# theAdamColton/spiht

Hardware: AMD Instinct MI355X
Metric: Mpixels/sec encode+decode at fixed bpp; bitstream-exact vs Rust ref (higher is better)
Workload: dtype f64 DWT / int32 bit-plane coding; 1 GPU; cfg2 image (1920x1080 RGB, bior2.2 reflect level 7, q=50, 0.5 bpp) x 256 per GPU (cfg4 shard), encode+decode, HBM-resident; images_per_gpu=256, distinct_images_per_gpu=256, seeds=1000 + global image index, streams=1, images_per_launch=256, decoder_waves=8, max_bits=1036800

## Files before the change

include/spiht_hip.h:

```cpp
#ifndef SPIHT_HIP_H
#define SPIHT_HIP_H

#include <stdint.h>

#ifdef __cplusplus
extern "C" {
#endif

enum {
    SPIHT_OK = 0,
    SPIHT_ERR_LL = 1,
    SPIHT_ERR_EMPTY = 2,
    SPIHT_ERR_SHAPE = 3,
    SPIHT_ERR_CAPACITY = 4,
    SPIHT_ERR_HIP = 5,
    SPIHT_ERR_ARG = 6,
    SPIHT_ERR_MAGNITUDE = 7,
    SPIHT_ERR_INTERNAL = 8,
    SPIHT_ERR_TOO_LARGE = 9,
    SPIHT_ERR_NOMEM = 10
};

enum { SPIHT_MODE_REFLECT = 0, SPIHT_MODE_SYMMETRIC = 1, SPIHT_MODE_PERIODIC = 2, SPIHT_MODE_ZERO = 3,
       SPIHT_MODE_CONSTANT = 4,
// ... 389 lines not shown
int spiht_convert_batch_flt(spiht_ctx *ctx, int kind, const double *d_in, int64_t B, int64_t c, int64_t rec_h, int64_t rec_w,
                            int64_t H, int64_t W, void *d_out, const int64_t *out_strides);
int spiht_decode_image_batch_flt(spiht_ctx *ctx, int kind, const uint8_t *d_data, uint64_t slot_stride, const uint64_t *d_nbytes,
                                 const uint8_t *d_max_n, int64_t B, int64_t c, int64_t H, int64_t W, int wavelet, int mode,
                                 int level, double q_scale, const double *channel_mults, void *d_img_out,
                                 const int64_t *out_strides, int32_t *d_rec);
int spiht_decode_image_host_flt(spiht_ctx *ctx, int kind, const uint8_t *data, uint64_t nbytes, uint8_t n, int64_t c, int64_t H,
                                int64_t W, int wavelet, int mode, int level, double q_scale, const double *channel_mults,
                                void *img_out, const int64_t *strides);
int spiht_dequant_idwt_flags_batch_flt(spiht_ctx *ctx, int kind, const int32_t *d_rec, const uint32_t *d_flags, int64_t B,
                                       int64_t c, int64_t H, int64_t W, int wavelet, int mode, int level, double q_scale,
                                       const double *channel_mults, void *d_img_out, const int64_t *out_strides);
int spiht_dequant_idwt_reduced_batch_flt(spiht_ctx *ctx, int kind, const int32_t *d_rec, int64_t B, int64_t c, int64_t H,
                                         int64_t W, int wavelet, int mode, int level, double q_scale,
                                         const double *channel_mults, void *d_img_out, const int64_t *out_strides, int reduce);
int spiht_decode_image_reduced_batch_flt(spiht_ctx *ctx, int kind, const uint8_t *d_data, uint64_t slot_stride,
                                         const uint64_t *d_nbytes, const uint8_t *d_max_n, int64_t B, int64_t c, int64_t H,
                                         int64_t W, int wavelet, int mode, int level, double q_scale,
                                         const double *channel_mults, void *d_img_out, const int64_t *out_strides,
                                         int32_t *d_rec, int reduce);
int spiht_decode_image_reduced_host_flt(spiht_ctx *ctx, int kind, const uint8_t *data, uint64_t nbytes, uint8_t n, int64_t c,
                                        int64_t H, int64_t W, int wavelet, int mode, int level, double q_scale,
                                        const double *channel_mults, void *img_out, const int64_t *strides, int reduce);
int spiht_tile_paste_f32s(spiht_ctx *ctx, const float *d_tiles, int64_t c, int64_t rh, int64_t rw, int64_t H, int64_t W,
                          int64_t th, int64_t tw, int64_t i0, int64_t i1, int64_t j0, int64_t j1, int64_t y0, int64_t x0,
                          int64_t wh, int64_t ww, float *d_out, const int64_t *out_strides);
int spiht_tile_mosaic_f32(spiht_ctx *ctx, const float *d_tiles, int64_t c, int64_t rh, int64_t rw, int64_t oy, int64_t ox,
                          int64_t H, int64_t W, int64_t th, int64_t tw, int64_t i0, int64_t i1, int64_t j0, int64_t j1,
                          int64_t y0, int64_t x0, int64_t wh, int64_t ww, float *d_out, const int64_t *out_strides);
int spiht_tile_blend_flt(spiht_ctx *ctx, int kind, const double *d_tiles, int64_t c, int64_t rh, int64_t rw, int64_t H, int64_t W,
                         int64_t th, int64_t tw, int64_t m, int64_t i0, int64_t i1, int64_t j0, int64_t j1, int64_t y0,
                         int64_t x0, int64_t wh, int64_t ww, void *d_out, const int64_t *out_strides);

#ifdef __cplusplus
}
#endif
#endif
```

spiht_amd/_lib.py:

```python
import ctypes as C
import os
import threading

_HERE = os.path.dirname(os.path.abspath(__file__))
LIB_PATH = os.environ.get("SPIHT_HIP_LIB") or os.path.join(_HERE, "libspiht_hip.so")

OK, ERR_LL, ERR_EMPTY, ERR_SHAPE, ERR_CAPACITY, ERR_HIP, ERR_ARG, ERR_MAGNITUDE, ERR_INTERNAL, ERR_TOO_LARGE, \
    ERR_NOMEM = range(11)

MODES = {"reflect": 0, "symmetric": 1, "periodic": 2, "zero": 3, "constant": 4}


class SpihtHipError(RuntimeError):
    """A HIP runtime failure or an internal guard of libspiht_hip."""


class PanicException(BaseException):
    """Counterpart of pyo3_runtime.PanicException, which the reference raises when the Rust core panics
    (assert!(ll_h > 1), encoder_decoder.rs:160-161; out-of-bounds index; unwrap on an empty array).
    Like PyO3's, it derives from BaseException."""


_lib = None
_lib_lock = threading.Lock()
# ... 12 lines not shown
    "spiht_dev_upload", "spiht_dev_download", "spiht_dev_memset", "spiht_dev_copy",
    "spiht_idwt_coarse_batch_f64", "spiht_idwt_level1_batch_f64", "spiht_idwt_level1_flags_batch_f64", "spiht_idwt_approx_shape",
    "spiht_encode_image_host_f64", "spiht_encode_image_host_f32", "spiht_decode_image_host_f64",
    "spiht_dequant_idwt_host_f64",
    "spiht_comm_unique_id", "spiht_comm_create", "spiht_comm_destroy", "spiht_comm_info", "spiht_gather_streams", "spiht_gather_row_offsets",
    "spiht_comm_barrier", "spiht_comm_allreduce_max_f64", "spiht_rccl_library", "spiht_ctx_lock", "spiht_ctx_unlock",
    "spiht_pipeline_create", "spiht_pipeline_create_on", "spiht_pipeline_destroy", "spiht_pipeline_info", "spiht_pipeline_set_color3", "spiht_pipeline_submit",
    "spiht_pipeline_submit_gather", "spiht_pipeline_flush", "spiht_pipeline_synchronize", "spiht_pipeline_contexts",
    "spiht_geometry_mode", "spiht_wavelet_taps", "spiht_ctx_set_option", "spiht_ctx_get_option", "spiht_ctx_wide_stats", "spiht_l1_flags_words", "spiht_decode_lists_flags_batch_i32", "spiht_dequant_idwt_flags_batch_f64",
    "spiht_encode_image_batch_u8", "spiht_decode_image_batch_u8", "spiht_encode_image_host_u8", "spiht_decode_image_host_u8",
    "spiht_dwt_pyramid_batch_u8", "spiht_dequant_idwt_flags_batch_u8", "spiht_idwt_level1_flags_batch_u8", "spiht_pipeline_submit_u8",
    "spiht_check_view_u8", "spiht_decode_with_metadata_batch_i32",
    "spiht_encode_image_batch_u16", "spiht_decode_image_batch_u16", "spiht_encode_image_host_u16", "spiht_decode_image_host_u16",
    "spiht_dwt_pyramid_batch_u16", "spiht_dequant_idwt_flags_batch_u16", "spiht_idwt_level1_flags_batch_u16", "spiht_pipeline_submit_u16",
    "spiht_check_view_u16",
    "spiht_reduced_shape",
    "spiht_dequant_idwt_reduced_batch_f64", "spiht_dequant_idwt_reduced_batch_u8", "spiht_dequant_idwt_reduced_batch_u16",
    "spiht_decode_image_reduced_batch_f64", "spiht_decode_image_reduced_batch_u8", "spiht_decode_image_reduced_batch_u16",
    "spiht_decode_image_reduced_host_f64", "spiht_decode_image_reduced_host_u8", "spiht_decode_image_reduced_host_u16",
    "spiht_sqerr_i32", "spiht_sse_f64", "spiht_sse_u8", "spiht_sse_u16",
    "spiht_tile_grid", "spiht_tile_cut_u8", "spiht_tile_cut_u16", "spiht_tile_cut_f32", "spiht_tile_cut_f64",
    "spiht_tile_paste_u8", "spiht_tile_paste_u16", "spiht_tile_paste_f32", "spiht_tile_paste_f64",
    "spiht_tile_pack", "spiht_tile_unpack",
    "spiht_tile_reduced_grid", "spiht_tile_mosaic_u8", "spiht_tile_mosaic_u16", "spiht_tile_mosaic_f64",
    "spiht_tile_prefix_slots", "spiht_sse_tiles_f64", "spiht_sse_tiles_u8", "spiht_sse_tiles_u16", "spiht_tile_allocate",
    "spiht_layer_pack", "spiht_layer_unpack",
    "spiht_sse_tiles_w_f64", "spiht_sse_tiles_w_u8", "spiht_sse_tiles_w_u16",
    "spiht_tile_allocate_target",
    "spiht_tile_cut_overlap_u8", "spiht_tile_cut_overlap_u16", "spiht_tile_cut_overlap_f32", "spiht_tile_cut_overlap_f64",
    "spiht_tile_blend_u8", "spiht_tile_blend_u16", "spiht_tile_blend_f64",
    "spiht_check_view_flt", "spiht_convert_batch_flt", "spiht_decode_image_batch_flt", "spiht_decode_image_host_flt",
    "spiht_dequant_idwt_flags_batch_flt", "spiht_dequant_idwt_reduced_batch_flt", "spiht_decode_image_reduced_batch_flt",
    "spiht_decode_image_reduced_host_flt", "spiht_tile_blend_flt", "spiht_tile_paste_f32s", "spiht_tile_mosaic_f32",
]


def lib():
    global _lib
    with _lib_lock:
        if _lib is not None:
            return _lib
        if not os.path.exists(LIB_PATH):
            raise ImportError(
                "libspiht_hip.so is missing (%s): build it with `python -c 'import __graft_entry__ as g; g.build()'` "
                "or `make -C spiht_amd/csrc`; spiht_amd has no CPU fallback" % LIB_PATH)
        try:
            L = C.CDLL(LIB_PATH)
        except OSError as e:
            raise ImportError("cannot load %s: %s" % (LIB_PATH, e))
        i64, u64, u8, i32 = C.c_int64, C.c_uint64, C.c_uint8, C.c_int
        vp = C.c_void_p
        L.spiht_strerror.restype = C.c_char_p
        L.spiht_strerror.argtypes = [i32]
        L.spiht_last_hip_error.restype = C.c_char_p
        L.spiht_ctx_create.argtypes = [i32, C.POINTER(vp)]
        L.spiht_ctx_create_priority.argtypes = [i32, i32, C.POINTER(vp)]
        L.spiht_ctx_resident_ticket.argtypes = [vp, C.POINTER(vp), C.POINTER(C.c_uint32)]
        L.spiht_ctx_wait_resident.argtypes = [vp, vp, C.c_uint32, C.c_uint32]
        L.spiht_ctx_destroy.argtypes = [vp]
        L.spiht_ctx_destroy.restype = None
        L.spiht_ctx_synchronize.argtypes = [vp]
        L.spiht_ctx_wait_on.argtypes = [vp, vp]
        L.spiht_event_create.argtypes = [vp, C.POINTER(vp)]
        L.spiht_event_destroy.argtypes = [vp]
        L.spiht_event_destroy.restype = None
        L.spiht_event_record.argtypes = [vp, vp]
# ... 322 lines not shown
```

spiht_amd/csrc/common.h:

```cpp
#pragma once
#include <hip/hip_runtime.h>
#include <stdint.h>

#define SPIHT_MAX_LEVELS 32
#define SPIHT_MAX_TAPS 20

struct FastDiv {
    uint32_t m, sh, d, pad;
};

static inline FastDiv fastdiv_make(uint32_t d) {
    FastDiv f;
    f.d = d;
    f.pad = 0;
    if (d < 2) { f.m = 0; f.sh = 0; return f; }
    uint32_t l = 0;
    while ((1ull << l) < d) l++;
    uint64_t m = ((1ull << 32) * ((1ull << l) - d)) / d + 1;
    f.m = (uint32_t)m;
    f.sh = l - 1;
    return f;
}

#ifdef __HIPCC__
__device__ __forceinline__ uint32_t fdiv(uint32_t n, const FastDiv &f) {
    uint32_t t = __umulhi(f.m, n);
    return (t + ((n - t) >> 1)) >> f.sh;
}
#endif

struct Geom {
    int32_t c, h, w, ll_h, ll_w;
    uint32_t hw;
    uint32_t n;
    uint32_t pad;
    FastDiv div_w, div_hw;
};

#define ENT_A 0x80000000u
#define ENT_LEAF 0x40000000u
#define ENT_IDX 0x3FFFFFFFu

struct ListCaps {
    uint32_t lip, lsp, lis;
    uint32_t pad;
};

struct WideCtl {
    uint32_t bar_count, bar_gen;
    uint32_t go;
    uint32_t bad;
    uint32_t st[12];
    uint32_t tot[8];
    uint32_t bad_at;
    uint32_t pad[3];
};
struct WideArgs {
    WideCtl *ctl;
    uint64_t *desc;
    uint32_t maxchunks;
// ... 107 lines not shown
    double A[9], M[9], p;
};

struct PxView {
    const uint8_t *in;
    uint8_t *out;
    int64_t sb, sc, sh, sw;
    int32_t c, h, w;
    int32_t es;
    int32_t kind;
    int32_t pad;
};

struct DwtKArgs {
    int32_t c;
    int32_t F, mode;
    int32_t in_h, in_w, out_h, out_w;
    int32_t off_h, off_w, enc_h, enc_w;
    int32_t last;
    int32_t planes;
    int32_t f32;
    int32_t ov_h, ov_w;
    const double *in;
    double *ll_out;
    int32_t *coeffs;
    const double *mults;
    uint32_t *maxabs;
    double q;
    double lo[SPIHT_MAX_TAPS], hi[SPIHT_MAX_TAPS];
    float lo_f[SPIHT_MAX_TAPS], hi_f[SPIHT_MAX_TAPS];
    int32_t color, pad2;
    Color3 col;
    PxView px;
};

struct TileCtr {
    uint32_t *dev;
    uint32_t base[8];
    int32_t wg_per_cu;
    int32_t num_cu;
    int32_t lds_per_cu;
    uint32_t started;
};
#define TILECTR_WORDS (9 * 32)
#define TILECTR_STARTED (8 * 32)
struct TileBase { uint32_t v[8]; };

struct IdwtKArgs {
    int32_t c;
    int32_t F;
    int32_t band_h, band_w;
    int32_t out_h, out_w;
    int32_t a_h, a_w;
    int32_t off_h, off_w, enc_h, enc_w;
    int32_t first;
    int32_t planes;
    const double *a_in;
    const int32_t *rec;
    const uint32_t *flags;
    double *out;
    const double *mults;
    double q;
    double lo[SPIHT_MAX_TAPS], hi[SPIHT_MAX_TAPS];
    int32_t color, pad2;
    Color3 col;
    PxView px;
};
// ... 12 lines not shown
```

spiht_amd/csrc/dwt.hip:

```cpp
#include "common.h"
#include "floatpx.h"
#include <stdlib.h>
#include <string.h>

#include <algorithm>

#ifndef DW_TH
#define DW_TH 12
#endif
#define DW32_TH 16
#ifndef DW_TW
#define DW_TW 64
#endif
#define DW_BLOCK 256
#ifndef DWF_BLOCK
#define DWF_BLOCK 192
#endif

__device__ __forceinline__ void xcd_tile_at(uint32_t L, uint32_t gx, uint32_t gy, uint32_t gz, uint32_t &bx, uint32_t &by,
                                            uint32_t &bz) {
    const uint32_t nt = gx * gy * gz;
    const uint32_t q = nt >> 3, r = nt & 7u, x = L & 7u, j = L >> 3;
    const uint32_t T = x * q + (x < r ? x : r) + j;
    bx = T % gx;
    const uint32_t t2 = T / gx;
    by = t2 % gy;
    bz = t2 / gy;
}

__device__ __forceinline__ void xcd_tile(uint32_t gx, uint32_t gy, uint32_t gz, uint32_t &bx, uint32_t &by, uint32_t &bz) {
    xcd_tile_at(blockIdx.x, gx, gy, gz, bx, by, bz);
}

__device__ __forceinline__ void block_raise_max(uint32_t *p, uint32_t v, uint32_t *s_m) {
    for (int o = 32; o > 0; o >>= 1) v = max(v, (uint32_t)__shfl_xor((int)v, o));
    if ((threadIdx.x & 63) == 0 && v) atomicMax(s_m, v);
    __syncthreads();
    if (threadIdx.x == 0) {
        const uint32_t m = *s_m;
        if (m > __hip_atomic_load(p, __ATOMIC_RELAXED, __HIP_MEMORY_SCOPE_WORKGROUP)) atomicMax(p, m);
    }
}

__device__ __forceinline__ void wave_raise_max(uint32_t *maxabs, int img, uint32_t v) {
    const int any = __builtin_amdgcn_readfirstlane(__builtin_amdgcn_readlane(img, __builtin_ctzll(__ballot(img >= 0) | (1ull << 63))));
    if (__ballot(img >= 0) == 0) return;
    if (__all(img < 0 || img == any)) {
        for (int o = 32; o > 0; o >>= 1) v = max(v, (uint32_t)__shfl_xor((int)v, o));
        if ((threadIdx.x & 63) == 0 && v > __hip_atomic_load(&maxabs[any], __ATOMIC_RELAXED, __HIP_MEMORY_SCOPE_AGENT))
            atomicMax(&maxabs[any], v);
    } else if (img >= 0 && v) {
        atomicMax(&maxabs[img], v);
    }
}

__device__ __forceinline__ int ext_index(int i, int N, int mode) {
    if (i >= 0 && i < N) return i;
    switch (mode) {
    case 0: {
        if (N == 1) return 0;
        int P = 2 * (N - 1);
        int m = i % P; if (m < 0) m += P;
        return m < N ? m : P - m;
    }
    case 1: {
        int P = 2 * N;
        int m = i % P; if (m < 0) m += P;
        return m < N ? m : P - 1 - m;
    }
    case 2: {
        int m = i % N; if (m < 0) m += N;
        return m;
    }
    case 4: return i < 0 ? 0 : N - 1;
    default: return -1;
    }
}

__device__ __forceinline__ int32_t quant(double v, double m, double q, bool has_m) {
    if (has_m) v = m * v;
    v = v * q;
    return (int32_t)v;
}
__device__ __forceinline__ uint32_t iabs_u(int32_t x) { return (uint32_t)(x < 0 ? -x : x); }
__device__ __forceinline__ double dequant(int32_t r, double m, double q, bool has_m) {
    double v = (double)r;
    if (has_m) v = v / m;
    return v / q;
}

__device__ __forceinline__ double px8_value(uint8_t k) {
    const double x = (double)k, r = 1.0 / 255.0;
    const double q = x * r;
    return fma(fma(-q, 255.0, x), r, q);
}
__device__ __forceinline__ uint8_t px8_store_value(double v) {
    const double c = fmin(fmax(v, 0.0), 1.0);
    const double s = c * 255.0;
    return (uint8_t)(uint32_t)s;
}
__device__ __forceinline__ double px16_value(uint16_t k) {
    const double x = (double)k, r = 1.0 / 65535.0;
    const double q = x * r;
    return fma(fma(-q, 65535.0, x), r, q);
}
__device__ __forceinline__ uint16_t px16_store_value(double v) {
    const double c = fmin(fmax(v, 0.0), 1.0);
    const double s = c * 65535.0;
    return (uint16_t)(uint32_t)s;
}
enum PxKind : int { PX_F64 = 0, PX_U8 = 1, PX_U16 = 2, PX_FLT = 3 };
static inline int px_kind_of(const PxView &px) { return px.kind ? PX_FLT : px.es == 2 ? PX_U16 : PX_U8; }
__device__ __forceinline__ void flt_store(uint8_t *p, double v, int kind) {
    const uint32_t b = flt_store_value(v, kind);
    if (kind == SPIHT_FLT_F32) *reinterpret_cast<uint32_t *>(p) = b;
    else *reinterpret_cast<uint16_t *>(p) = (uint16_t)b;
}
template <int PX> __device__ __forceinline__ uint32_t px_load(const uint8_t *p) {
    if constexpr (PX == PX_U16) return *reinterpret_cast<const uint16_t *>(p);
    else return *p;
}
template <int PX> __device__ __forceinline__ double px_value(uint32_t raw) {
    if constexpr (PX == PX_U16) return px16_value((uint16_t)raw);
    else return px8_value((uint8_t)raw);
}
#define PX_STORE(PX, p, o, v, kind)                                                         \
    do {                                                                                    \
        if constexpr ((PX) == PX_FLT) flt_store((p) + (o), v, kind);                        \
        else if constexpr ((PX) == PX_U16) *reinterpret_cast<uint16_t *>((p) + (o)) = px16_store_value(v); \
        else (p)[o] = px8_store_value(v);                                                   \
    } while (0)

template <int F, uint32_t LOM, uint32_t HIM, int PS, int NR, int PX = PX_F64>
__device__ __forceinline__ void dwt_tile(const DwtKArgs &a, double (&s_lo)[2][PS], double (&s_hi)[2][PS], uint32_t tbx, uint32_t tby,
                                         uint32_t tbz) {
    constexpr int NC = 2 * DW_TW + F - 2;
    constexpr int HC = (NC + 1) / 2;
    static_assert(NC <= DWF_BLOCK, "one thread per input column");
    static_assert(NR == 2 * DW_TH + F - 2, "input rows needed");
    constexpr int RS = HC + 1;
    const int plane = (int)tbz;
    const int oh0 = (int)tby * DW_TH, ow0 = (int)tbx * DW_TW;
    const double *__restrict__ in = PX ? nullptr : a.in + (size_t)plane * a.in_h * a.in_w;
    const uint8_t *__restrict__ in8 = PX ? a.px.in + (int64_t)(plane / a.c) * a.px.sb + (int64_t)(plane % a.c) * a.px.sc : nullptr;
    const int tid = threadIdx.x;

    const int r0 = 2 * oh0 + 2 - F, c0 = 2 * ow0 + 2 - F;
    __shared__ long long s_off[NR];
    if (tid < NR) {
        const int gr = ext_index(r0 + tid, a.in_h, a.mode);
        s_off[tid] = gr < 0 ? -1ll : (long long)gr * (PX ? a.px.sh : (long long)a.in_w);
    }
    __shared__ uint32_t s_amax;
    if (tid == 0) s_amax = 0;
    __syncthreads();

    if (tid < NC) {
        const int gc = ext_index(c0 + tid, a.in_w, a.mode);
        double x[NR];
        int lz = 0;
        asm volatile("" : "+v"(lz));
        if (PX) {
            const long long co8 = gc < 0 ? 0 : (long long)gc * a.px.sw;
            uint32_t raw[NR];
            static_assert(NR <= 64, "one bit per row");
            uint64_t okm = 0;
#pragma unroll
            for (int r = 0; r < NR; r++) {
                const long long off = s_off[r + lz];
                const bool ok = a.mode != 3 || (gc >= 0 && off >= 0);
                okm |= (ok ? 1ull : 0ull) << r;
                raw[r] = px_load<PX>(in8 + (ok ? off + co8 : 0));
            }
#pragma unroll
            for (int r = 0; r < NR; r++) x[r] = ((okm >> r) & 1ull) ? px_value<PX>(raw[r]) : 0.0;
        } else if (a.mode != 3) {
#pragma unroll
            for (int r = 0; r < NR; r++) x[r] = in[s_off[r + lz] + gc];
        } else {
#pragma unroll
            for (int r = 0; r < NR; r++) {
                const long long off = s_off[r + lz];
                const bool ok = gc >= 0 && off >= 0;
                const double v = in[ok ? off + gc : 0];
                x[r] = ok ? v : 0.0;
            }
        }
        const int par = tid & 1, hc = tid >> 1;
#pragma unroll
        for (int o = 0; o < DW_TH; o++) {
            double sl = 0.0, shh = 0.0;
#pragma unroll
            for (int j = 0; j < F; j++) {
                if ((LOM >> j) & 1u) sl += a.lo[j] * x[2 * o + F - 1 - j];
                if ((HIM >> j) & 1u) shh += a.hi[j] * x[2 * o + F - 1 - j];
            }
            s_lo[par][o * RS + hc] = sl;
            s_hi[par][o * RS + hc] = shh;
        }
    }
    __syncthreads();

    const int k = plane % a.c;
    const bool has_m = a.mults != nullptr;
    const double mk = has_m ? a.mults[k] : 1.0;
    int32_t *__restrict__ co = a.coeffs + (size_t)plane * a.enc_h * a.enc_w;
    double *__restrict__ llo = a.last ? nullptr : a.ll_out + (size_t)plane * a.out_h * a.out_w;
    uint32_t amax = 0;
    constexpr int NU = (DW_TH * DW_TW + DWF_BLOCK - 1) / DWF_BLOCK;
#pragma unroll
    for (int u = 0; u < NU; u++) {
        const int p = tid + u * DWF_BLOCK;
        const int o = p / DW_TW, wcol = p % DW_TW;
        const int oh = oh0 + o, ow = ow0 + wcol;
        if (o >= DW_TH || oh >= a.out_h || ow >= a.out_w) continue;
        double aa = 0.0, ad = 0.0, da = 0.0, dd = 0.0;
#pragma unroll
        for (int j = 0; j < F; j++) {
            const double vl = s_lo[(F - 1 - j) & 1][o * RS + wcol + ((F - 1 - j) >> 1)];
            const double vh = s_hi[(F - 1 - j) & 1][o * RS + wcol + ((F - 1 - j) >> 1)];
            if ((LOM >> j) & 1u) { aa += a.lo[j] * vl; da += a.lo[j] * vh; }
            if ((HIM >> j) & 1u) { ad += a.hi[j] * vl; dd += a.hi[j] * vh; }
        }
        const int32_t qad = quant(ad, mk, a.q, has_m), qda = quant(da, mk, a.q, has_m), qdd = quant(dd, mk, a.q, has_m);
        const bool mine = oh < a.ov_h && ow < a.ov_w;
        if (a.last) {
            const int32_t qaa = quant(aa, mk, a.q, has_m);
            co[(size_t)oh * a.enc_w + ow] = qaa;
            if (mine) amax = max(amax, iabs_u(qaa));
        } else {
            llo[(size_t)oh * a.out_w + ow] = aa;
        }
        co[(size_t)oh * a.enc_w + a.off_w + ow] = qad;
        co[(size_t)(a.off_h + oh) * a.enc_w + ow] = qda;
        co[(size_t)(a.off_h + oh) * a.enc_w + a.off_w + ow] = qdd;
        if (mine) amax = max(amax, max(iabs_u(qad), max(iabs_u(qda), iabs_u(qdd))));
    }
    if (a.maxabs != nullptr) {
        block_raise_max(&a.maxabs[plane / a.c], amax, &s_amax);
    }
}

template <int F, uint32_t LOM, uint32_t HIM, int PX = PX_F64>
__global__ __launch_bounds__(DWF_BLOCK) void k_dwt_level(DwtKArgs a) {
    constexpr int NC = 2 * DW_TW + F - 2, NR = 2 * DW_TH + F - 2, HC = (NC + 1) / 2;
    constexpr int RS = HC + 1, PS = DW_TH * RS + (24 - (DW_TH * RS) % 16) % 16;
    __shared__ double s_lo[2][PS];
    __shared__ double s_hi[2][PS];
    uint32_t tbx, tby, tbz;
    uint32_t lin = blockIdx.x;
    asm volatile("" : "+v"(lin));
    xcd_tile_at(lin, (a.out_w + DW_TW - 1) / DW_TW, (a.out_h + DW_TH - 1) / DW_TH, a.planes, tbx, tby, tbz);
    dwt_tile<F, LOM, HIM, PS, NR, PX>(a, s_lo, s_hi, tbx, tby, tbz);
}

typedef unsigned int u32x2 __attribute__((ext_vector_type(2)));
__device__ __forceinline__ void lds_barrier() { asm volatile("s_waitcnt lgkmcnt(0)\n\ts_barrier" ::: "memory"); }
#define BUF_OOB 0x80000000u
__device__ __forceinline__ __amdgpu_buffer_rsrc_t plane_rsrc(const void *p, uint32_t bytes) {
    const uint64_t v = (uint64_t)p;
    const uint32_t lo = __builtin_amdgcn_readfirstlane((uint32_t)v), hi = __builtin_amdgcn_readfirstlane((uint32_t)(v >> 32));
    return __builtin_amdgcn_make_buffer_rsrc((void *)(((uint64_t)hi << 32) | lo), 0, (int)__builtin_amdgcn_readfirstlane(bytes),
                                             0x00020000);
}

template <int F, int PX = PX_F64>
__global__ __launch_bounds__(256) void k_dwt_edge(DwtKArgs a) {
    __shared__ double s_f[2][F];
    if (threadIdx.x < F) { s_f[0][threadIdx.x] = a.lo[threadIdx.x]; s_f[1][threadIdx.x] = a.hi[threadIdx.x]; }
    __shared__ uint32_t s_amax;
    if (threadIdx.x == 0) s_amax = 0;
    __syncthreads();
    const int nr = a.out_h - a.ov_h, nc = a.out_w - a.ov_w;
    const int nA = nr * a.out_w, total = nA + a.ov_h * nc;
    const int t = blockIdx.x * 256 + threadIdx.x;
    const int plane = blockIdx.y;
    uint32_t amax = 0;
    if (t < total) {
        int oh, ow;
        if (t < nA) { oh = a.ov_h + t / a.out_w; ow = t % a.out_w; }
        else { const int u = t - nA; oh = u / nc; ow = a.ov_w + u % nc; }
        const double *__restrict__ in = PX ? nullptr : a.in + (size_t)plane * a.in_h * a.in_w;
        const uint8_t *__restrict__ in8 = PX ? a.px.in + (int64_t)(plane / a.c) * a.px.sb + (int64_t)(plane % a.c) * a.px.sc : nullptr;
        const int ir = 2 * oh + 1, ic = 2 * ow + 1;
        const int jbr = oh >= a.ov_h ? ir - a.in_h : -1, jbc = ow >= a.ov_w ? ic - a.in_w : -1;
        int gr[F];
#pragma unroll
        for (int r = 0; r < F; r++) gr[r] = ext_index(ir - r, a.in_h, a.mode);
        double aa = 0.0, ad = 0.0, da = 0.0, dd = 0.0;
#pragma unroll F <= 6 ? F : 1
        for (int s1 = 0; s1 < F; s1++) {
            const int j = s1 <= jbc ? jbc - s1 : s1;
            const int gc = ext_index(ic - j, a.in_w, a.mode);
            double xv[F];
#pragma unroll
            for (int r = 0; r < F; r++) {
// ... 1052 lines not shown
#pragma unroll
                for (int ch = 0; ch < 3; ch++) {
                    double sa = 0.0, sd = 0.0;
#pragma unroll
                    for (int j = 0; j < HF; j++) {
                        const int s = HF - 1 - j;
                        const bool lnz = (LOM >> (mp + F - 2 - 2 * s)) & 1u, hnz = (HIM >> (mp + F - 2 - 2 * s)) & 1u;
                        if (lnz) sa += wl[ch][s] * a.lo[mp + F - 2 - 2 * s];
                        if (hnz) sd += wh[ch][s] * a.hi[mp + F - 2 - 2 * s];
                    }
                    px[ch] = (0.0 + sa) + sd;
                }
                if (PX ? (m + mp < a.px.h && n < a.px.w) : (m + mp < a.out_h && n < a.out_w)) {
                    double w0, w1, w2;
                    color3_px(a.col, s_pw, px[0], px[1], px[2], w0, w1, w2);
                    if (PX) {
                        const int64_t o = (int64_t)(m + mp) * a.px.sh + (int64_t)n * a.px.sw;
                        PX_STORE(PX, out8, o, w0, a.px.kind);
                        PX_STORE(PX, out8, o + a.px.sc, w1, a.px.kind);
                        PX_STORE(PX, out8, o + 2 * a.px.sc, w2, a.px.kind);
                    } else {
                        const size_t o = (size_t)(m + mp) * a.out_w + n;
                        out[o] = w0;
                        out[o + opl] = w1;
                        out[o + 2 * opl] = w2;
                    }
                }
            }
        }
    }
}


template <int F, uint32_t LOM, uint32_t HIM>
static int launch_dwt_FM(DwtKArgs a, int planes, hipStream_t st) {
    a.planes = planes;
    const int px = a.px.in == nullptr ? PX_F64 : a.px.es == 2 ? PX_U16 : PX_U8;
    a.ov_h = a.out_h;
    a.ov_w = a.out_w;
    if (a.f32) {
        uint32_t ntf = (uint32_t)((a.out_w + DW_TW - 1) / DW_TW) * (uint32_t)((a.out_h + DW32_TH - 1) / DW32_TH) * (uint32_t)planes;
        hipLaunchKernelGGL((k_dwt_level_f32<F, LOM, HIM>), dim3(ntf), dim3(DW_BLOCK), 0, st, a);
        return (int)hipGetLastError();
    }
    if (a.color) {
        constexpr int SW = (256 - (F - 2)) / 2;
        int z = 0;
        while (z < F && a.lo[z] == 0.0 && a.hi[z] == 0.0) z++;
        if (a.mode != 4) a.ov_h = min(a.out_h, (a.in_h + z + 2) / 2);
        if (a.mode != 4) a.ov_w = min(a.out_w, (a.in_w + z + 2) / 2);
        const uint32_t gx = (uint32_t)((a.out_w + SW - 1) / SW), gy = (uint32_t)((a.out_h + C1_ROWS - 1) / C1_ROWS);
        if (px == PX_U16) hipLaunchKernelGGL((k_dwt1_color<F, LOM, HIM, PX_U16>), dim3(gx * gy * (uint32_t)(planes / 3)), dim3(256), 0, st, a, gx, gy);
        else if (px == PX_U8) hipLaunchKernelGGL((k_dwt1_color<F, LOM, HIM, PX_U8>), dim3(gx * gy * (uint32_t)(planes / 3)), dim3(256), 0, st, a, gx, gy);
        else hipLaunchKernelGGL((k_dwt1_color<F, LOM, HIM>), dim3(gx * gy * (uint32_t)(planes / 3)), dim3(256), 0, st, a, gx, gy);
        return (int)hipGetLastError();
    }
    int z = 0;
    while (z < F && a.lo[z] == 0.0 && a.hi[z] == 0.0) z++;
    if (a.mode != 4) a.ov_h = min(a.out_h, (a.in_h + z + 2) / 2);
    if (a.mode != 4) a.ov_w = min(a.out_w, (a.in_w + z + 2) / 2);
    const uint32_t nt = (uint32_t)((a.out_w + DW_TW - 1) / DW_TW) * (uint32_t)((a.out_h + DW_TH - 1) / DW_TH) * (uint32_t)planes;
    if (px == PX_U16) hipLaunchKernelGGL((k_dwt_level<F, LOM, HIM, PX_U16>), dim3(nt), dim3(DWF_BLOCK), 0, st, a);
    else if (px == PX_U8) hipLaunchKernelGGL((k_dwt_level<F, LOM, HIM, PX_U8>), dim3(nt), dim3(DWF_BLOCK), 0, st, a);
    else hipLaunchKernelGGL((k_dwt_level<F, LOM, HIM>), dim3(nt), dim3(DWF_BLOCK), 0, st, a);
    const int n_edge = (a.out_h - a.ov_h) * a.out_w + a.ov_h * (a.out_w - a.ov_w);
    if (n_edge > 0) {
        if (px == PX_U16) hipLaunchKernelGGL((k_dwt_edge<F, PX_U16>), dim3((n_edge + 255) / 256, planes), dim3(256), 0, st, a);
        else if (px == PX_U8) hipLaunchKernelGGL((k_dwt_edge<F, PX_U8>), dim3((n_edge + 255) / 256, planes), dim3(256), 0, st, a);
        else hipLaunchKernelGGL(k_dwt_edge<F>, dim3((n_edge + 255) / 256, planes), dim3(256), 0, st, a);
    }
    return (int)hipGetLastError();
}
template <int F, uint32_t LOM, uint32_t HIM>
static int launch_dwt_F(const DwtKArgs &a, int planes, hipStream_t st) {
    uint32_t lom = 0, him = 0;
    for (int j = 0; j < F; j++) {
        if (a.lo[j] != 0.0) lom |= 1u << j;
        if (a.hi[j] != 0.0) him |= 1u << j;
    }
    if (lom == LOM && him == HIM) return launch_dwt_FM<F, LOM, HIM>(a, planes, st);
    return launch_dwt_FM<F, (1u << F) - 1u, (1u << F) - 1u>(a, planes, st);
}
template <int F, uint32_t LOM, uint32_t HIM, int PX>
static void launch_idwt_pf(IdwtKArgs &a, uint32_t G, uint32_t pad, hipStream_t st, uint32_t gx, uint32_t gy, uint32_t *ctr, const TileBase &cb) {
    if (a.first) hipLaunchKernelGGL((k_idwt_level_pf<F, LOM, HIM, true, false, PX>), dim3(G), dim3(DW_BLOCK), pad, st, a, gx, gy, ctr, cb);
    else if (a.flags && (uint64_t)a.enc_h * a.enc_w * 4u < (1ull << 31))
        hipLaunchKernelGGL((k_idwt_level_pf<F, LOM, HIM, false, true, PX>), dim3(G), dim3(DW_BLOCK), pad, st, a, gx, gy, ctr, cb);
    else { a.flags = nullptr; hipLaunchKernelGGL((k_idwt_level_pf<F, LOM, HIM, false, false, PX>), dim3(G), dim3(DW_BLOCK), pad, st, a, gx, gy, ctr, cb); }
}
template <int F, uint32_t LOM, uint32_t HIM>
static int launch_idwt_FM(IdwtKArgs a, int planes, hipStream_t st, TileCtr *tc) {
    a.planes = planes;
    const int px = a.px.out == nullptr ? PX_F64 : px_kind_of(a.px);
    if (a.color) {
        uint32_t ntc = (uint32_t)((a.out_w + IW_TW - 1) / IW_TW) * (uint32_t)((a.out_h + IWC_TH - 1) / IWC_TH) * (uint32_t)(planes / 3);
        if (px == PX_FLT) hipLaunchKernelGGL((k_idwt1_color<F, LOM, HIM, PX_FLT>), dim3(ntc), dim3(DW_BLOCK), 0, st, a);
        else if (px == PX_U16) hipLaunchKernelGGL((k_idwt1_color<F, LOM, HIM, PX_U16>), dim3(ntc), dim3(DW_BLOCK), 0, st, a);
// ... 199 lines not shown
```

Before: 32910 Mpixels/s.

## Use 32-bit buffer addressing and fast division in forward DWT level kernel

```diff
diff --git a/include/spiht_hip.h b/include/spiht_hip.h
--- a/include/spiht_hip.h
+++ b/include/spiht_hip.h
@@ -445,6 +445,9 @@
                          int64_t th, int64_t tw, int64_t m, int64_t i0, int64_t i1, int64_t j0, int64_t j1, int64_t y0,
                          int64_t x0, int64_t wh, int64_t ww, void *d_out, const int64_t *out_strides);
 
+int spiht_dwt_addr32(int64_t in_h, int64_t in_w, int64_t out_h, int64_t out_w, int64_t enc_h, int64_t enc_w, int px_es,
+                     int64_t px_sh, int64_t px_sw);
+
 #ifdef __cplusplus
 }
 #endif
diff --git a/spiht_amd/_lib.py b/spiht_amd/_lib.py
--- a/spiht_amd/_lib.py
+++ b/spiht_amd/_lib.py
@@ -68,6 +68,7 @@
     "spiht_check_view_flt", "spiht_convert_batch_flt", "spiht_decode_image_batch_flt", "spiht_decode_image_host_flt",
     "spiht_dequant_idwt_flags_batch_flt", "spiht_dequant_idwt_reduced_batch_flt", "spiht_decode_image_reduced_batch_flt",
     "spiht_decode_image_reduced_host_flt", "spiht_tile_blend_flt", "spiht_tile_paste_f32s", "spiht_tile_mosaic_f32",
+    "spiht_dwt_addr32",
 ]
 
 
diff --git a/spiht_amd/csrc/common.h b/spiht_amd/csrc/common.h
--- a/spiht_amd/csrc/common.h
+++ b/spiht_amd/csrc/common.h
@@ -26,6 +26,33 @@
 __device__ __forceinline__ uint32_t fdiv(uint32_t n, const FastDiv &f) {
     uint32_t t = __umulhi(f.m, n);
     return (t + ((n - t) >> 1)) >> f.sh;
+}
+#endif
+
+struct FastDivU {
+    uint32_t m, s1, s2, d;
+};
+
+static inline FastDivU fastdivu_make(uint32_t d) {
+    FastDivU f;
+    if (d < 1) d = 1;
+    f.d = d;
+    uint32_t l = 0;
+    while ((1ull << l) < d) l++;
+    f.m = (uint32_t)(((1ull << 32) * ((1ull << l) - d)) / d + 1);
+    f.s1 = l < 1 ? l : 1;
+    f.s2 = l < 1 ? 0 : l - 1;
+    return f;
+}
+static inline uint32_t fastdivu_host(uint32_t n, const FastDivU &f) {
+    const uint32_t t = (uint32_t)(((uint64_t)f.m * n) >> 32);
+    return (t + ((n - t) >> f.s1)) >> f.s2;
+}
+
+#ifdef __HIPCC__
+__device__ __forceinline__ uint32_t fdivu(uint32_t n, const FastDivU &f) {
+    const uint32_t t = __umulhi(f.m, n);
+    return (t + ((n - t) >> f.s1)) >> f.s2;
 }
 #endif
 
@@ -199,7 +226,30 @@
     int32_t color, pad2;
     Color3 col;
     PxView px;
-};
+    FastDivU dv_gx, dv_gy, dv_c;
+    uint32_t gx, gy, nt;
+    int32_t narrow;
+    uint32_t in_pb;
+    uint32_t in_rb, in_cb;
+    uint32_t co_pb, co_rb;
+    uint32_t ll_pb, ll_rb;
+    uint32_t pad3;
+};
+
+static inline bool dwt_narrow_ok(int64_t in_h, int64_t in_w, int64_t out_h, int64_t out_w, int64_t enc_h, int64_t enc_w, int px_es,
+                                 int64_t px_sh, int64_t px_sw) {
+    const int64_t lim = (int64_t)1 << 30;
+    if (in_h < 1 || in_w < 1 || out_h < 1 || out_w < 1 || enc_h < 1 || enc_w < 1) return false;
+    if (in_h >= lim || in_w >= lim || out_h >= lim / 16 || out_w >= lim / 16 || enc_h >= lim || enc_w >= lim) return false;
+    if (px_es) {
+        if (px_sh < 0 || px_sw < 0 || px_sh >= lim || px_sw >= lim) return false;
+        if ((in_h - 1) * px_sh + (in_w - 1) * px_sw + px_es >= lim) return false;
+    } else if (in_h * in_w * 8 >= lim) return false;
+    if (enc_h * enc_w * 4 >= lim) return false;
+    if (out_h * out_w * 8 >= lim) return false;
+    if ((out_h + 64) * enc_w * 4 >= 2 * lim || (out_h + 64) * out_w * 8 >= 2 * lim) return false;
+    return true;
+}
 
 struct TileCtr {
     uint32_t *dev;
diff --git a/spiht_amd/csrc/dwt.hip b/spiht_amd/csrc/dwt.hip
--- a/spiht_amd/csrc/dwt.hip
+++ b/spiht_amd/csrc/dwt.hip
@@ -13,6 +13,9 @@
 #define DW_TW 64
 #endif
 #define DW_BLOCK 256
+#ifndef DWF_STRAY
+#define DWF_STRAY 1
+#endif
 #ifndef DWF_BLOCK
 #define DWF_BLOCK 192
 #endif
@@ -32,9 +35,19 @@
     xcd_tile_at(blockIdx.x, gx, gy, gz, bx, by, bz);
 }
 
+#define DPP_MAX_STEP(v, ctrl, rows) v = max(v, (uint32_t)__builtin_amdgcn_update_dpp(0, (int)(v), ctrl, rows, 0xF, false))
+__device__ __forceinline__ uint32_t wave_max_lane63(uint32_t v) {
+    DPP_MAX_STEP(v, 0xB1, 0xF);
+    DPP_MAX_STEP(v, 0x4E, 0xF);
+    DPP_MAX_STEP(v, 0x141, 0xF);
+    DPP_MAX_STEP(v, 0x140, 0xF);
+    DPP_MAX_STEP(v, 0x142, 0xA);
+    DPP_MAX_STEP(v, 0x143, 0xC);
+    return v;
+}
 __device__ __forceinline__ void block_raise_max(uint32_t *p, uint32_t v, uint32_t *s_m) {
-    for (int o = 32; o > 0; o >>= 1) v = max(v, (uint32_t)__shfl_xor((int)v, o));
-    if ((threadIdx.x & 63) == 0 && v) atomicMax(s_m, v);
+    v = wave_max_lane63(v);
+    if ((threadIdx.x & 63) == 63 && v) atomicMax(s_m, v);
     __syncthreads();
     if (threadIdx.x == 0) {
         const uint32_t m = *s_m;
@@ -54,23 +67,30 @@
     }
 }
 
+__device__ __forceinline__ int ext_mod(int i, int P) {
+    int m = i < 0 ? i + P : i;
+    if (m >= P) m -= P;
+    if ((unsigned)m >= (unsigned)P) {
+        m = i % P; if (m < 0) m += P;
+    }
+    return m;
+}
 __device__ __forceinline__ int ext_index(int i, int N, int mode) {
     if (i >= 0 && i < N) return i;
     switch (mode) {
     case 0: {
         if (N == 1) return 0;
         int P = 2 * (N - 1);
-        int m = i % P; if (m < 0) m += P;
+        int m = ext_mod(i, P);
         return m < N ? m : P - m;
     }
     case 1: {
         int P = 2 * N;
-        int m = i % P; if (m < 0) m += P;
+        int m = ext_mod(i, P);
         return m < N ? m : P - 1 - m;
     }
     case 2: {
-        int m = i % N; if (m < 0) m += N;
-        return m;
+        return ext_mod(i, N);
     }
     case 4: return i < 0 ? 0 : N - 1;
     default: return -1;
@@ -131,59 +151,156 @@
         else (p)[o] = px8_store_value(v);                                                   \
     } while (0)
 
-template <int F, uint32_t LOM, uint32_t HIM, int PS, int NR, int PX = PX_F64>
+typedef unsigned int u32x2 __attribute__((ext_vector_type(2)));
+__device__ __forceinline__ void lds_barrier() { asm volatile("s_waitcnt lgkmcnt(0)\n\ts_barrier" ::: "memory"); }
+#define BUF_OOB 0x80000000u
+__device__ __forceinline__ __amdgpu_buffer_rsrc_t plane_rsrc(const void *p, uint32_t bytes) {
+    const uint64_t v = (uint64_t)p;
+    const uint32_t lo = __builtin_amdgcn_readfirstlane((uint32_t)v), hi = __builtin_amdgcn_readfirstlane((uint32_t)(v >> 32));
+    return __builtin_amdgcn_make_buffer_rsrc((void *)(((uint64_t)hi << 32) | lo), 0, (int)__builtin_amdgcn_readfirstlane(bytes),
+                                             0x00020000);
+}
+
+__device__ __forceinline__ void xcd_tile_fd(uint32_t L, const DwtKArgs &a, uint32_t &bx, uint32_t &by, uint32_t &bz) {
+    const uint32_t q = a.nt >> 3, r = a.nt & 7u, x = L & 7u, j = L >> 3;
+    const uint32_t T = x * q + (x < r ? x : r) + j;
+    const uint32_t t2 = fdivu(T, a.dv_gx);
+    bx = T - t2 * a.gx;
+    bz = fdivu(t2, a.dv_gy);
+    by = t2 - bz * a.gy;
+}
+#define OOB_ROW BUF_OOB
+#define OOB_COL 0x40000000u
+
+template <int F, uint32_t LOM, uint32_t HIM, int PS, int NR, int PX = PX_F64, bool WIDE = false>
 __device__ __forceinline__ void dwt_tile(const DwtKArgs &a, double (&s_lo)[2][PS], double (&s_hi)[2][PS], uint32_t tbx, uint32_t tby,
                                          uint32_t tbz) {
     constexpr int NC = 2 * DW_TW + F - 2;
     constexpr int HC = (NC + 1) / 2;
     static_assert(NC <= DWF_BLOCK, "one thread per input column");
     static_assert(NR == 2 * DW_TH + F - 2, "input rows needed");
+    static_assert(DW_TH <= 64, "dwt_narrow_ok allows for 64 rows below the level's last");
     constexpr int RS = HC + 1;
-    const int plane = (int)tbz;
+    constexpr int NRP = (NR + 3) & ~3;
+    const uint32_t plane = tbz;
+    const uint32_t img = fdivu(plane, a.dv_c), k = plane - img * (uint32_t)a.c;
     const int oh0 = (int)tby * DW_TH, ow0 = (int)tbx * DW_TW;
-    const double *__restrict__ in = PX ? nullptr : a.in + (size_t)plane * a.in_h * a.in_w;
-    const uint8_t *__restrict__ in8 = PX ? a.px.in + (int64_t)(plane / a.c) * a.px.sb + (int64_t)(plane % a.c) * a.px.sc : nullptr;
     const int tid = threadIdx.x;
 
     const int r0 = 2 * oh0 + 2 - F, c0 = 2 * ow0 + 2 - F;
-    __shared__ long long s_off[NR];
+    __shared__ __attribute__((aligned(16))) uint32_t s_off[WIDE ? 4 : NRP];
+    __shared__ long long s_off64[WIDE ? NR : 1];
     if (tid < NR) {
         const int gr = ext_index(r0 + tid, a.in_h, a.mode);
-        s_off[tid] = gr < 0 ? -1ll : (long long)gr * (PX ? a.px.sh : (long long)a.in_w);
+        if constexpr (WIDE) s_off64[tid] = gr < 0 ? -1ll : (long long)gr * (PX ? a.px.sh : (long long)a.in_w);
+        else s_off[tid] = gr < 0 ? OOB_ROW : (uint32_t)gr * a.in_rb;
     }
     __shared__ uint32_t s_amax;
     if (tid == 0) s_amax = 0;
     __syncthreads();
 
-    if (tid < NC) {
+    constexpr int NFULL = NC / 64 * 64, NS = NC - NFULL;
+    constexpr bool STRAY = DWF_STRAY && !WIDE && NS > 0 && NS * DW_TH <= 64;
+    if constexpr (STRAY) {
+        const int it = tid - NFULL;
+        if (it >= 0 && it < NS * DW_TH) {
+            const int o = it / NS, sc = NFULL + it % NS;
+            const int gc = ext_index(c0 + sc, a.in_w, a.mode);
+            const uint8_t *pb = PX ? a.px.in + (int64_t)img * a.px.sb + (int64_t)k * a.px.sc
+                                   : reinterpret_cast<const uint8_t *>(a.in) + (uint64_t)plane * a.in_pb;
+            const __amdgpu_buffer_rsrc_t rs_in = plane_rsrc(pb, a.in_pb);
+            const uint32_t cb = gc < 0 ? OOB_COL : (uint32_t)gc * (PX ? a.in_cb : 8u);
+            double x[F];
+            if constexpr (PX != PX_F64) {
+                uint32_t raw[F];
+#pragma unroll
+                for (int t = 0; t < F; t++) {
+                    if constexpr (PX == PX_U16) raw[t] = __builtin_amdgcn_raw_buffer_load_b16(rs_in, s_off[2 * o + t] + cb, 0, 0);
+                    else raw[t] = __builtin_amdgcn_raw_buffer_load_b8(rs_in, s_off[2 * o + t] + cb, 0, 0);
+                }
+#pragma unroll
+                for (int t = 0; t < F; t++) x[t] = px_value<PX>(raw[t]);
+            } else {
+#pragma unroll
+                for (int t = 0; t < F; t++)
+                    x[t] = __builtin_bit_cast(double, __builtin_amdgcn_raw_buffer_load_b64(rs_in, s_off[2 * o + t] + cb, 0, 0));
+            }
+            double sl = 0.0, shh = 0.0;
+#pragma unroll
+            for (int j = 0; j < F; j++) {
+                if ((LOM >> j) & 1u) sl += a.lo[j] * x[F - 1 - j];
+                if ((HIM >> j) & 1u) shh += a.hi[j] * x[F - 1 - j];
+            }
+            s_lo[sc & 1][o * RS + (sc >> 1)] = sl;
+            s_hi[sc & 1][o * RS + (sc >> 1)] = shh;
+        }
+    }
+    if (tid < (STRAY ? NFULL : NC)) {
         const int gc = ext_index(c0 + tid, a.in_w, a.mode);
         double x[NR];
         int lz = 0;
         asm volatile("" : "+v"(lz));
-        if (PX) {
-            const long long co8 = gc < 0 ? 0 : (long long)gc * a.px.sw;
-            uint32_t raw[NR];
-            static_assert(NR <= 64, "one bit per row");
-            uint64_t okm = 0;
-#pragma unroll
-            for (int r = 0; r < NR; r++) {
-                const long long off = s_off[r + lz];
-                const bool ok = a.mode != 3 || (gc >= 0 && off >= 0);
-                okm |= (ok ? 1ull : 0ull) << r;
-                raw[r] = px_load<PX>(in8 + (ok ? off + co8 : 0));
-            }
-#pragma unroll
-            for (int r = 0; r < NR; r++) x[r] = ((okm >> r) & 1ull) ? px_value<PX>(raw[r]) : 0.0;
-        } else if (a.mode != 3) {
-#pragma unroll
-            for (int r = 0; r < NR; r++) x[r] = in[s_off[r + lz] + gc];
+        if constexpr (!WIDE) {
+            const uint8_t *pb = PX ? a.px.in + (int64_t)img * a.px.sb + (int64_t)k * a.px.sc
+                                   : reinterpret_cast<const uint8_t *>(a.in) + (uint64_t)plane * a.in_pb;
+            const __amdgpu_buffer_rsrc_t rs_in = plane_rsrc(pb, a.in_pb);
+            const uint32_t cb = gc < 0 ? OOB_COL : (uint32_t)gc * (PX ? a.in_cb : 8u);
+            const uint4 *so = reinterpret_cast<const uint4 *>(s_off) + lz;
+            if constexpr (PX != PX_F64) {
+                uint32_t raw[NRP];
+#pragma unroll
+                for (int q = 0; q < NRP / 4; q++) {
+                    const uint4 o4 = so[q];
+                    const uint32_t o[4] = {o4.x, o4.y, o4.z, o4.w};
+#pragma unroll
+                    for (int e = 0; e < 4; e++) {
+                        if (4 * q + e >= NR) continue;
+                        if constexpr (PX == PX_U16) raw[4 * q + e] = __builtin_amdgcn_raw_buffer_load_b16(rs_in, o[e] + cb, 0, 0);
+                        else raw[4 * q + e] = __builtin_amdgcn_raw_buffer_load_b8(rs_in, o[e] + cb, 0, 0);
+                    }
+                }
+#pragma unroll
+                for (int r = 0; r < NR; r++) x[r] = px_value<PX>(raw[r]);
+            } else {
+#pragma unroll
+                for (int q = 0; q < NRP / 4; q++) {
+                    const uint4 o4 = so[q];
+                    const uint32_t o[4] = {o4.x, o4.y, o4.z, o4.w};
+#pragma unroll
+                    for (int e = 0; e < 4; e++) {
+                        if (4 * q + e >= NR) continue;
+                        x[4 * q + e] = __builtin_bit_cast(double, __builtin_amdgcn_raw_buffer_load_b64(rs_in, o[e] + cb, 0, 0));
+                    }
+                }
+            }
         } else {
-#pragma unroll
-            for (int r = 0; r < NR; r++) {
-                const long long off = s_off[r + lz];
-                const bool ok = gc >= 0 && off >= 0;
-                const double v = in[ok ? off + gc : 0];
-                x[r] = ok ? v : 0.0;
+            const double *__restrict__ in = PX ? nullptr : a.in + (size_t)plane * a.in_h * a.in_w;
+            const uint8_t *__restrict__ in8 = PX ? a.px.in + (int64_t)img * a.px.sb + (int64_t)k * a.px.sc : nullptr;
+            if (PX) {
+                const long long co8 = gc < 0 ? 0 : (long long)gc * a.px.sw;
+                uint32_t raw[NR];
+                static_assert(NR <= 64, "one bit per row");
+                uint64_t okm = 0;
+#pragma unroll
+                for (int r = 0; r < NR; r++) {
+                    const long long off = s_off64[r + lz];
+                    const bool ok = a.mode != 3 || (gc >= 0 && off >= 0);
+                    okm |= (ok ? 1ull : 0ull) << r;
+                    raw[r] = px_load<PX>(in8 + (ok ? off + co8 : 0));
+                }
+#pragma unroll
+                for (int r = 0; r < NR; r++) x[r] = ((okm >> r) & 1ull) ? px_value<PX>(raw[r]) : 0.0;
+            } else if (a.mode != 3) {
+#pragma unroll
+                for (int r = 0; r < NR; r++) x[r] = in[s_off64[r + lz] + gc];
+            } else {
+#pragma unroll
+                for (int r = 0; r < NR; r++) {
+                    const long long off = s_off64[r + lz];
+                    const bool ok = gc >= 0 && off >= 0;
+                    const double v = in[ok ? off + gc : 0];
+                    x[r] = ok ? v : 0.0;
+                }
             }
         }
         const int par = tid & 1, hc = tid >> 1;
@@ -201,47 +318,91 @@
     }
     __syncthreads();
 
-    const int k = plane % a.c;
     const bool has_m = a.mults != nullptr;
     const double mk = has_m ? a.mults[k] : 1.0;
-    int32_t *__restrict__ co = a.coeffs + (size_t)plane * a.enc_h * a.enc_w;
-    double *__restrict__ llo = a.last ? nullptr : a.ll_out + (size_t)plane * a.out_h * a.out_w;
     uint32_t amax = 0;
     constexpr int NU = (DW_TH * DW_TW + DWF_BLOCK - 1) / DWF_BLOCK;
-#pragma unroll
-    for (int u = 0; u < NU; u++) {
-        const int p = tid + u * DWF_BLOCK;
-        const int o = p / DW_TW, wcol = p % DW_TW;
-        const int oh = oh0 + o, ow = ow0 + wcol;
-        if (o >= DW_TH || oh >= a.out_h || ow >= a.out_w) continue;
-        double aa = 0.0, ad = 0.0, da = 0.0, dd = 0.0;
-#pragma unroll
-        for (int j = 0; j < F; j++) {
-            const double vl = s_lo[(F - 1 - j) & 1][o * RS + wcol + ((F - 1 - j) >> 1)];
-            const double vh = s_hi[(F - 1 - j) & 1][o * RS + wcol + ((F - 1 - j) >> 1)];
-            if ((LOM >> j) & 1u) { aa += a.lo[j] * vl; da += a.lo[j] * vh; }
-            if ((HIM >> j) & 1u) { ad += a.hi[j] * vl; dd += a.hi[j] * vh; }
-        }
-        const int32_t qad = quant(ad, mk, a.q, has_m), qda = quant(da, mk, a.q, has_m), qdd = quant(dd, mk, a.q, has_m);
-        const bool mine = oh < a.ov_h && ow < a.ov_w;
-        if (a.last) {
-            const int32_t qaa = quant(aa, mk, a.q, has_m);
-            co[(size_t)oh * a.enc_w + ow] = qaa;
-            if (mine) amax = max(amax, iabs_u(qaa));
-        } else {
-            llo[(size_t)oh * a.out_w + ow] = aa;
-        }
-        co[(size_t)oh * a.enc_w + a.off_w + ow] = qad;
-        co[(size_t)(a.off_h + oh) * a.enc_w + ow] = qda;
-        co[(size_t)(a.off_h + oh) * a.enc_w + a.off_w + ow] = qdd;
-        if (mine) amax = max(amax, max(iabs_u(qad), max(iabs_u(qda), iabs_u(qdd))));
+    if constexpr (!WIDE) {
+        static_assert(DWF_BLOCK % DW_TW == 0 && (DW_TH * DW_TW) % DWF_BLOCK == 0, "a thread keeps its column; whole steps");
+        constexpr int RSTEP = DWF_BLOCK / DW_TW;
+        const int o0 = tid / DW_TW, wcol = tid % DW_TW;
+        const int oh = oh0 + o0, ow = ow0 + wcol;
+        const bool colok = ow < a.out_w;
+        uint32_t vco = colok ? (uint32_t)oh * a.co_rb + (uint32_t)ow * 4u : BUF_OOB;
+        uint32_t vll = colok ? (uint32_t)oh * a.ll_rb + (uint32_t)ow * 8u : BUF_OOB;
+        uint8_t *cob = reinterpret_cast<uint8_t *>(a.coeffs) + (uint64_t)plane * a.co_pb;
+        const uint32_t band_bytes = (uint32_t)a.out_h * a.co_rb;
+        const __amdgpu_buffer_rsrc_t rs_top = plane_rsrc(cob, band_bytes);
+        const __amdgpu_buffer_rsrc_t rs_bot = plane_rsrc(cob + (uint64_t)(uint32_t)a.off_h * a.co_rb, band_bytes);
+        const __amdgpu_buffer_rsrc_t rs_ll =
+            plane_rsrc(reinterpret_cast<uint8_t *>(a.ll_out) + (uint64_t)plane * a.ll_pb, a.last ? 0u : (uint32_t)a.out_h * a.ll_rb);
+        const uint32_t so_w = (uint32_t)a.off_w * 4u;
+        const int mine_rows = ow < a.ov_w ? a.ov_h - oh : 0;
+#pragma unroll
+        for (int u = 0; u < NU; u++) {
+            const int o = o0 + u * RSTEP;
+            double aa = 0.0, ad = 0.0, da = 0.0, dd = 0.0;
+#pragma unroll
+            for (int j = 0; j < F; j++) {
+                const double vl = s_lo[(F - 1 - j) & 1][o * RS + wcol + ((F - 1 - j) >> 1)];
+                const double vh = s_hi[(F - 1 - j) & 1][o * RS + wcol + ((F - 1 - j) >> 1)];
+                if ((LOM >> j) & 1u) { aa += a.lo[j] * vl; da += a.lo[j] * vh; }
+                if ((HIM >> j) & 1u) { ad += a.hi[j] * vl; dd += a.hi[j] * vh; }
+            }
+            const int32_t qad = quant(ad, mk, a.q, true), qda = quant(da, mk, a.q, true), qdd = quant(dd, mk, a.q, true);
+            uint32_t m = max(iabs_u(qad), max(iabs_u(qda), iabs_u(qdd)));
+            if (a.last) {
+                const int32_t qaa = quant(aa, mk, a.q, true);
+                __builtin_amdgcn_raw_buffer_store_b32((uint32_t)qaa, rs_top, vco, 0, 0);
+                m = max(m, iabs_u(qaa));
+            } else {
+                __builtin_amdgcn_raw_buffer_store_b64(__builtin_bit_cast(u32x2, aa), rs_ll, vll, 0, 0);
+            }
+            __builtin_amdgcn_raw_buffer_store_b32((uint32_t)qad, rs_top, vco, so_w, 0);
+            __builtin_amdgcn_raw_buffer_store_b32((uint32_t)qda, rs_bot, vco, 0, 0);
+            __builtin_amdgcn_raw_buffer_store_b32((uint32_t)qdd, rs_bot, vco, so_w, 0);
+            amax = max(amax, u * RSTEP < mine_rows ? m : 0u);
+            vco += (uint32_t)RSTEP * a.co_rb;
+            vll += (uint32_t)RSTEP * a.ll_rb;
+        }
+    } else {
+        int32_t *__restrict__ co = a.coeffs + (size_t)plane * a.enc_h * a.enc_w;
+        double *__restrict__ llo = a.last ? nullptr : a.ll_out + (size_t)plane * a.out_h * a.out_w;
+#pragma unroll
+        for (int u = 0; u < NU; u++) {
+            const int p = tid + u * DWF_BLOCK;
+            const int o = p / DW_TW, wcol = p % DW_TW;
+            const int oh = oh0 + o, ow = ow0 + wcol;
+            if (o >= DW_TH || oh >= a.out_h || ow >= a.out_w) continue;
+            double aa = 0.0, ad = 0.0, da = 0.0, dd = 0.0;
+#pragma unroll
+            for (int j = 0; j < F; j++) {
+                const double vl = s_lo[(F - 1 - j) & 1][o * RS + wcol + ((F - 1 - j) >> 1)];
+                const double vh = s_hi[(F - 1 - j) & 1][o * RS + wcol + ((F - 1 - j) >> 1)];
+                if ((LOM >> j) & 1u) { aa += a.lo[j] * vl; da += a.lo[j] * vh; }
+                if ((HIM >> j) & 1u) { ad += a.hi[j] * vl; dd += a.hi[j] * vh; }
+            }
+            const int32_t qad = quant(ad, mk, a.q, has_m), qda = quant(da, mk, a.q, has_m), qdd = quant(dd, mk, a.q, has_m);
+            const bool mine = oh < a.ov_h && ow < a.ov_w;
+            if (a.last) {
+                const int32_t qaa = quant(aa, mk, a.q, has_m);
+                co[(size_t)oh * a.enc_w + ow] = qaa;
+                if (mine) amax = max(amax, iabs_u(qaa));
+            } else {
+                llo[(size_t)oh * a.out_w + ow] = aa;
+            }
+            co[(size_t)oh * a.enc_w + a.off_w + ow] = qad;
+            co[(size_t)(a.off_h + oh) * a.enc_w + ow] = qda;
+            co[(size_t)(a.off_h + oh) * a.enc_w + a.off_w + ow] = qdd;
+            if (mine) amax = max(amax, max(iabs_u(qad), max(iabs_u(qda), iabs_u(qdd))));
+        }
     }
     if (a.maxabs != nullptr) {
-        block_raise_max(&a.maxabs[plane / a.c], amax, &s_amax);
-    }
-}
-
-template <int F, uint32_t LOM, uint32_t HIM, int PX = PX_F64>
+        block_raise_max(&a.maxabs[img], amax, &s_amax);
+    }
+}
+
+template <int F, uint32_t LOM, uint32_t HIM, int PX = PX_F64, bool WIDE = false>
 __global__ __launch_bounds__(DWF_BLOCK) void k_dwt_level(DwtKArgs a) {
     constexpr int NC = 2 * DW_TW + F - 2, NR = 2 * DW_TH + F - 2, HC = (NC + 1) / 2;
     constexpr int RS = HC + 1, PS = DW_TH * RS + (24 - (DW_TH * RS) % 16) % 16;
@@ -250,18 +411,8 @@
     uint32_t tbx, tby, tbz;
     uint32_t lin = blockIdx.x;
     asm volatile("" : "+v"(lin));
-    xcd_tile_at(lin, (a.out_w + DW_TW - 1) / DW_TW, (a.out_h + DW_TH - 1) / DW_TH, a.planes, tbx, tby, tbz);
-    dwt_tile<F, LOM, HIM, PS, NR, PX>(a, s_lo, s_hi, tbx, tby, tbz);
-}
-
-typedef unsigned int u32x2 __attribute__((ext_vector_type(2)));
-__device__ __forceinline__ void lds_barrier() { asm volatile("s_waitcnt lgkmcnt(0)\n\ts_barrier" ::: "memory"); }
-#define BUF_OOB 0x80000000u
-__device__ __forceinline__ __amdgpu_buffer_rsrc_t plane_rsrc(const void *p, uint32_t bytes) {
-    const uint64_t v = (uint64_t)p;
-    const uint32_t lo = __builtin_amdgcn_readfirstlane((uint32_t)v), hi = __builtin_amdgcn_readfirstlane((uint32_t)(v >> 32));
-    return __builtin_amdgcn_make_buffer_rsrc((void *)(((uint64_t)hi << 32) | lo), 0, (int)__builtin_amdgcn_readfirstlane(bytes),
-                                             0x00020000);
+    xcd_tile_fd(lin, a, tbx, tby, tbz);
+    dwt_tile<F, LOM, HIM, PS, NR, PX, WIDE>(a, s_lo, s_hi, tbx, tby, tbz);
 }
 
 template <int F, int PX = PX_F64>
@@ -1380,6 +1531,32 @@
 }
 
 
+extern "C" int spiht_dwt_addr32(int64_t in_h, int64_t in_w, int64_t out_h, int64_t out_w, int64_t enc_h, int64_t enc_w, int px_es,
+                                int64_t px_sh, int64_t px_sw) {
+    return dwt_narrow_ok(in_h, in_w, out_h, out_w, enc_h, enc_w, px_es, px_sh, px_sw) ? 1 : 0;
+}
+static uint32_t dwt_set_launch_consts(DwtKArgs &a, int planes, int px) {
+    a.gx = (uint32_t)((a.out_w + DW_TW - 1) / DW_TW);
+    a.gy = (uint32_t)((a.out_h + DW_TH - 1) / DW_TH);
+    a.nt = a.gx * a.gy * (uint32_t)planes;
+    a.dv_gx = fastdivu_make(a.gx);
+    a.dv_gy = fastdivu_make(a.gy);
+    a.dv_c = fastdivu_make((uint32_t)a.c);
+    const char *force = getenv("SPIHT_DWT_ADDR64");
+    a.narrow = spiht_dwt_addr32(a.in_h, a.in_w, a.out_h, a.out_w, a.enc_h, a.enc_w, px ? a.px.es : 0, a.px.sh, a.px.sw) &&
+               !(force && atoi(force) != 0);
+    if (a.narrow) {
+        a.in_pb = px ? (uint32_t)((a.in_h - 1) * a.px.sh + (a.in_w - 1) * a.px.sw + a.px.es) : (uint32_t)a.in_h * (uint32_t)a.in_w * 8u;
+        a.in_rb = px ? (uint32_t)a.px.sh : (uint32_t)a.in_w * 8u;
+        a.in_cb = px ? (uint32_t)a.px.sw : 8u;
+        a.co_pb = (uint32_t)a.enc_h * (uint32_t)a.enc_w * 4u;
+        a.co_rb = (uint32_t)a.enc_w * 4u;
+        a.ll_pb = (uint32_t)a.out_h * (uint32_t)a.out_w * 8u;
+        a.ll_rb = (uint32_t)a.out_w * 8u;
+    }
+    return a.nt;
+}
+
 template <int F, uint32_t LOM, uint32_t HIM>
 static int launch_dwt_FM(DwtKArgs a, int planes, hipStream_t st) {
     a.planes = planes;
@@ -1407,10 +1584,16 @@
     while (z < F && a.lo[z] == 0.0 && a.hi[z] == 0.0) z++;
     if (a.mode != 4) a.ov_h = min(a.out_h, (a.in_h + z + 2) / 2);
     if (a.mode != 4) a.ov_w = min(a.out_w, (a.in_w + z + 2) / 2);
-    const uint32_t nt = (uint32_t)((a.out_w + DW_TW - 1) / DW_TW) * (uint32_t)((a.out_h + DW_TH - 1) / DW_TH) * (uint32_t)planes;
-    if (px == PX_U16) hipLaunchKernelGGL((k_dwt_level<F, LOM, HIM, PX_U16>), dim3(nt), dim3(DWF_BLOCK), 0, st, a);
-    else if (px == PX_U8) hipLaunchKernelGGL((k_dwt_level<F, LOM, HIM, PX_U8>), dim3(nt), dim3(DWF_BLOCK), 0, st, a);
-    else hipLaunchKernelGGL((k_dwt_level<F, LOM, HIM>), dim3(nt), dim3(DWF_BLOCK), 0, st, a);
+    const uint32_t nt = dwt_set_launch_consts(a, planes, px);
+    if (a.narrow) {
+        if (px == PX_U16) hipLaunchKernelGGL((k_dwt_level<F, LOM, HIM, PX_U16>), dim3(nt), dim3(DWF_BLOCK), 0, st, a);
+        else if (px == PX_U8) hipLaunchKernelGGL((k_dwt_level<F, LOM, HIM, PX_U8>), dim3(nt), dim3(DWF_BLOCK), 0, st, a);
+        else hipLaunchKernelGGL((k_dwt_level<F, LOM, HIM>), dim3(nt), dim3(DWF_BLOCK), 0, st, a);
+    } else {
+        if (px == PX_U16) hipLaunchKernelGGL((k_dwt_level<F, LOM, HIM, PX_U16, true>), dim3(nt), dim3(DWF_BLOCK), 0, st, a);
+        else if (px == PX_U8) hipLaunchKernelGGL((k_dwt_level<F, LOM, HIM, PX_U8, true>), dim3(nt), dim3(DWF_BLOCK), 0, st, a);
+        else hipLaunchKernelGGL((k_dwt_level<F, LOM, HIM, PX_F64, true>), dim3(nt), dim3(DWF_BLOCK), 0, st, a);
+    }
     const int n_edge = (a.out_h - a.ov_h) * a.out_w + a.ov_h * (a.out_w - a.ov_w);
     if (n_edge > 0) {
         if (px == PX_U16) hipLaunchKernelGGL((k_dwt_edge<F, PX_U16>), dim3((n_edge + 255) / 256, planes), dim3(256), 0, st, a);
```

Measured after the change: 33860 Mpixels/s, median of 6. +2.9%, better.
